# Moryu-Io/Roboken-FMSKF-robot-controller

Measured on NVIDIA B200. Metric: robot-instance control steps/sec, higher is better.
Workload: dtype f32

## Files before the change

### roboken-fmskf-robot-controller_b200/csrc/rk_imu.cu

```cuda
#include <string.h>

#include "rk_common.cuh"
#include "rk_math.cuh"
#include "rk_stream.cuh"

namespace rk {

struct ImuData {
  float d[16];
};

RK_DEV void cvt2_s16(uint32_t w, float &lo, float &hi) {
  asm("{ .reg .b16 l, h; mov.b32 {l, h}, %2; cvt.rn.f32.s16 %0, l; cvt.rn.f32.s16 %1, h; }" : "=f"(lo), "=f"(hi) : "r"(w));
}
struct ImuQ {
  float2 a[4], b[4];
};
RK_DEV void imu_q_pairs(ImuQ &k, const float qi[4]) {
  k.a[0] = make_float2(qi[3], -qi[2]), k.a[1] = make_float2(qi[2], qi[3]), k.a[2] = make_float2(-qi[1], qi[0]), k.a[3] = make_float2(-qi[0], -qi[1]);
  k.b[0] = make_float2(qi[1], qi[0]), k.b[1] = make_float2(-qi[0], qi[1]), k.b[2] = make_float2(qi[3], qi[2]), k.b[3] = make_float2(-qi[2], qi[3]);
}
RK_DEV float2 imu_mul2(float s, float2 k, float nz) { return __ffma2_rn(make_float2(s, s), k, make_float2(nz, nz)); }
RK_DEV void imu_update_data_w(const ImuQ &k, const uint32_t rw[8], float nz, ImuData &o) {
  float f[16];
#pragma unroll
  for(int j = 0; j < 8; j++) cvt2_s16(rw[j], f[2 * j], f[2 * j + 1]);
  const float KA = 16.0f / 32768.0f, KG = 2000.0f / 32768.0f, KE = 180.0f / 32768.0f, S = 1.0f / 32768.0f;
  o.d[0] = fmul(f[0], KA), o.d[1] = fmul(f[1], -KA), o.d[2] = fmul(f[2], -KA);
  o.d[3] = fmul(f[3], KG), o.d[4] = fmul(f[4], -KG), o.d[5] = fmul(f[5], -KG);
  o.d[6] = f[6], o.d[7] = -f[7], o.d[8] = -f[8];
  o.d[9]  = fsub(normalize_deg_0to360(fmul(f[9], KE)), 180.0f);
  o.d[10] = fmul(f[10], KE);
  o.d[11] = fmul(f[11], KE);
  float q[4];
#pragma unroll
  for(int j = 0; j < 4; j++) q[j] = fmul(f[12 + j], S);
  const float2 ra = __fadd2_rn(__fadd2_rn(__fadd2_rn(imu_mul2(q[0], k.a[0], nz), imu_mul2(q[1], k.a[1], nz)), imu_mul2(q[2], k.a[2], nz)),
                               imu_mul2(q[3], k.a[3], nz));
  const float2 rb = __fadd2_rn(__fadd2_rn(__fadd2_rn(imu_mul2(q[0], k.b[0], nz), imu_mul2(q[1], k.b[1], nz)), imu_mul2(q[2], k.b[2], nz)),
                               imu_mul2(q[3], k.b[3], nz));
  o.d[14] = -ra.x, o.d[13] = ra.y, o.d[12] = -rb.x, o.d[15] = rb.y;
}

template <bool OUT, bool YAW, bool GEN>
RK_DEV void imt_update_body(int64_t i, uint4 *__restrict__ state, int64_t n, int K, const int16_t *__restrict__ regs,
                            const uint8_t *__restrict__ have_quat, float4 *__restrict__ out, float *__restrict__ yaw_rad, int do_init,
                            float nz, const rk_stream_desc_t &sd) {
  float   qi[4];
  ImuData cur;
  {
    const uint4 q = ld_plane(state, n, 0, i);
    qi[0] = u2f(q.x), qi[1] = u2f(q.y), qi[2] = u2f(q.z), qi[3] = u2f(q.w);
#pragma unroll
    for(int pl = 0; pl < 4; pl++) {
      const uint4 v = ld_plane(state, n, 1 + pl, i);
      cur.d[4 * pl] = u2f(v.x), cur.d[4 * pl + 1] = u2f(v.y), cur.d[4 * pl + 2] = u2f(v.z), cur.d[4 * pl + 3] = u2f(v.w);
    }
  }
  uint32_t flags = ld_plane(state, n, 5, i).x;
  const uint4   *src = (const uint4 *)regs + i;
  const uint8_t *hsrc = have_quat ? have_quat + i : nullptr;
  uint4          c0 = make_uint4(0u, 0u, 0u, 0u), c1 = c0;
  bool           nhq = true;
  const uint32_t px  = GEN ? h32_prefix(sd.seed, 20u, (uint64_t)(sd.first + i)) : 0u;
  uint32_t       upd = sd.first_update;
  auto           fetch = [&]() {
    if(GEN) {
      stream_imu_sample(px, upd++, sd.drop_every, c0, c1, nhq);
    } else {
      c0 = __ldcs(src), c1 = __ldcs(src + n);
      src += 2 * n;
      if(hsrc) nhq = __ldcs(hsrc) != 0, hsrc += n;
    }
  };
  auto publish = [&](int u) {
    if(YAW) __stcs(yaw_rad + (int64_t)u * n + i, fmul(cur.d[RK_IS_D_ANGLE + 2], RK_DEG2RAD));
    if(OUT) {
#pragma unroll
      for(int pl = 0; pl < 4; pl++)
        __stcs(out + ((int64_t)u * 4 + pl) * n + i, make_float4(cur.d[4 * pl], cur.d[4 * pl + 1], cur.d[4 * pl + 2], cur.d[4 * pl + 3]));
    }
  };
  if(K > 0) fetch();
  ImuQ kq;
  imu_q_pairs(kq, qi);
  int u = 0;
  if(do_init && K > 0) {
    const uint32_t rw[8] = {c0.x, c0.y, c0.z, c0.w, c1.x, c1.y, c1.z, c1.w};
    if(K > 1) fetch();
    imu_update_data_w(kq, rw, nz, cur);
    cvt2_s16(rw[6], qi[0], qi[1]), cvt2_s16(rw[7], qi[2], qi[3]);
#pragma unroll
    for(int j = 0; j < 4; j++) qi[j] = fmul(qi[j], 1.0f / 32768.0f);
    imu_q_pairs(kq, qi);
    publish(0);
    u = 1;
  }
  for(; u < K; u++) {
    const uint32_t rw[8] = {c0.x, c0.y, c0.z, c0.w, c1.x, c1.y, c1.z, c1.w};
    const bool     hq    = nhq;
    if(u + 1 < K) fetch();
    if(hq) {
      flags &= ~RK_IS_FLAG_ERROR;
      imu_update_data_w(kq, rw, nz, cur);
    } else {
      flags |= RK_IS_FLAG_ERROR;
    }
    publish(u);
  }
  st_plane(state, n, 0, i, make_uint4(f2u(qi[0]), f2u(qi[1]), f2u(qi[2]), f2u(qi[3])));
#pragma unroll
  for(int pl = 0; pl < 4; pl++)
    st_plane(state, n, 1 + pl, i, make_uint4(f2u(cur.d[4 * pl]), f2u(cur.d[4 * pl + 1]), f2u(cur.d[4 * pl + 2]), f2u(cur.d[4 * pl + 3])));
  st_plane(state, n, 5, i, make_uint4(flags, 0u, 0u, 0u));
}
template <bool OUT, bool YAW, bool GEN = false>
__global__ void __launch_bounds__(256, 4)
imt_update_kernel(uint4 *__restrict__ state, int64_t n, int K, const int16_t *__restrict__ regs,
                  const uint8_t *__restrict__ have_quat, float4 *__restrict__ out, float *__restrict__ yaw_rad, int do_init, float nz_src,
                  const rk_stream_desc_t *__restrict__ desc) {
  const float            nz = fmul(-0.0f, nz_src);
  const rk_stream_desc_t sd = GEN ? *desc : rk_stream_desc_t{};
  for(int64_t i = (int64_t)blockIdx.x * blockDim.x + threadIdx.x; i < n; i += (int64_t)gridDim.x * blockDim.x)
    imt_update_body<OUT, YAW, GEN>(i, state, n, K, regs, have_quat, out, yaw_rad, do_init, nz, sd);
}

struct Wit {
  uint32_t w0, w1, w2, cnt, flags;
  bool     head_ok;
  uint32_t rw[8];
};
RK_DEV void wit_push(Wit &p, uint32_t R, uint32_t k) {
  const uint32_t s = 8u * k;
  p.w0 = __funnelshift_rc(p.w0, p.w1, s);
  p.w1 = __funnelshift_rc(p.w1, p.w2, s);
  p.w2 = __funnelshift_rc(p.w2, R, s);
}
RK_DEV bool wit_head_is_55(const Wit &p) {
  const uint32_t off = 12u - p.cnt, w = off < 4u ? p.w0 : (off < 8u ? p.w1 : p.w2);
  return ((w >> (8u * (off & 3u))) & 0xFFu) == 0x55u;
}
RK_DEV void wit_store_reg(Wit &p, uint32_t reg, uint32_t val) {
  const uint32_t slot = (reg >= 0x34u && reg <= 0x3Fu) ? reg - 0x34u : ((reg >= 0x51u && reg <= 0x54u) ? reg - 0x51u + 12u : 0xFFu);
#pragma unroll
  for(int k = 0; k < 8; k++) {
    if(slot == 2u * k) p.rw[k] = __byte_perm(p.rw[k], val, 0x3254);
    if(slot == 2u * k + 1u) p.rw[k] = __byte_perm(p.rw[k], val, 0x5410);
  }
  if(reg == 0x54u) p.flags |= 1u;
}
RK_DEV void wit_dispatch(Wit &p, uint32_t type, uint32_t d01, uint32_t d23) {
  const bool acc = type == 0x51u, gyr = type == 0x52u, ang = type == 0x53u, mag = type == 0x54u, qut = type == 0x59u;
  const uint32_t d12 = __byte_perm(d01, d23, 0x5432);
  p.rw[0] = acc ? d01 : p.rw[0];
  p.rw[1] = acc ? __byte_perm(p.rw[1], d23, 0x3254) : (gyr ? __byte_perm(p.rw[1], d01, 0x5410) : p.rw[1]);
  p.rw[2] = gyr ? d12 : p.rw[2];
  p.rw[3] = mag ? d01 : p.rw[3];
  p.rw[4] = mag ? __byte_perm(p.rw[4], d23, 0x3254) : (ang ? __byte_perm(p.rw[4], d01, 0x5410) : p.rw[4]);
  p.rw[5] = ang ? d12 : p.rw[5];
  p.rw[6] = qut ? d01 : p.rw[6];
  p.rw[7] = qut ? d23 : p.rw[7];
  p.flags |= qut ? 1u : 0u;
  if(type == 0x5Fu) {
    const uint32_t r = (p.flags >> 8) & 0xFFu;
    wit_store_reg(p, r, d01 & 0xFFFFu), wit_store_reg(p, r + 1, d01 >> 16), wit_store_reg(p, r + 2, d23 & 0xFFFFu), wit_store_reg(p, r + 3, d23 >> 16);
  }
}
RK_DEV void wit_frame(Wit &p) {
  const uint32_t f0 = __funnelshift_r(p.w0, p.w1, 8), f1 = __funnelshift_r(p.w1, p.w2, 8), f2 = p.w2 >> 8;
  wit_dispatch(p, (f0 >> 8) & 0xFFu, __byte_perm(f0, f1, 0x5432), __byte_perm(f1, f2, 0x5432));
}
RK_DEV bool wit_try_frame(Wit &p, uint32_t f0, uint32_t f1, uint32_t f2) {
  if((f0 & 0xFFu) != 0x55u) return false;
  const uint32_t sum = __vsadu4(f0, 0u) + __vsadu4(f1, 0u) + __vsadu4(f2 & 0xFFFFu, 0u);
  if((sum & 0xFFu) != ((f2 >> 16) & 0xFFu)) return false;
  wit_dispatch(p, (f0 >> 8) & 0xFFu, __byte_perm(f0, f1, 0x5432), __byte_perm(f1, f2, 0x5432));
  return true;
}
RK_DEV void wit_bytes(Wit &p, uint32_t R, uint32_t rem) {
  while(rem) {
    if(p.cnt == 0u) p.head_ok = (R & 0xFFu) == 0x55u;
    if(p.head_ok) {
      const uint32_t take = min(rem, 11u - p.cnt);
      wit_push(p, R, take);
      p.cnt += take;
      R = __funnelshift_rc(R, 0u, 8u * take);
      rem -= take;
      if(p.cnt == 11u) {
        const uint32_t sum = __vsadu4(p.w0 & 0xFFFFFF00u, 0u) + __vsadu4(p.w1, 0u) + __vsadu4(p.w2 & 0x00FFFFFFu, 0u);
        if((sum & 0xFFu) == (p.w2 >> 24)) {
          wit_frame(p);
          p.cnt = 0u;
        } else {
          p.cnt     = 10u;
          p.head_ok = ((p.w0 >> 16) & 0xFFu) == 0x55u;
        }
      }
    } else {
      if(p.cnt) {
        wit_push(p, R, 1u);
        p.head_ok = wit_head_is_55(p);
      }
      R >>= 8;
      rem--;
    }
  }
}
RK_DEV void wit_load(Wit &p, const uint4 a) {
  p.cnt = min(a.z >> 24, 10u);
  p.w0 = a.x, p.w1 = a.y, p.w2 = a.z & 0x00FFFFFFu, p.flags = a.w;
  p.head_ok = p.cnt && (p.w0 & 0xFFu) == 0x55u;
  for(uint32_t k = p.cnt; k < 12u; k++) {
    p.w2 = __funnelshift_l(p.w1, p.w2, 8);
    p.w1 = __funnelshift_l(p.w0, p.w1, 8);
    p.w0 <<= 8;
  }
}
RK_DEV uint4 wit_save(const Wit &p) {
  uint32_t w0 = p.w0, w1 = p.w1, w2 = p.w2;
  for(uint32_t k = p.cnt; k < 12u; k++) {
    w0 = __funnelshift_r(w0, w1, 8);
    w1 = __funnelshift_r(w1, w2, 8);
    w2 >>= 8;
  }
  return make_uint4(w0, w1, w2 | (p.cnt << 24), p.flags);
}

RK_DEV uint32_t smem_u32(const void *p) { return (uint32_t)__cvta_generic_to_shared(p); }
RK_DEV void mbar_init(uint64_t *bar, uint32_t count) { asm volatile("mbarrier.init.shared::cta.b64 [%0], %1;" ::"r"(smem_u32(bar)), "r"(count) : "memory"); }
RK_DEV void mbar_fence_init() { asm volatile("fence.mbarrier_init.release.cluster;" ::: "memory"); }
RK_DEV void mbar_arrive(uint64_t *bar) { asm volatile("mbarrier.arrive.shared::cta.b64 _, [%0];" ::"r"(smem_u32(bar)) : "memory"); }
RK_DEV void mbar_arrive_expect_tx(uint64_t *bar, uint32_t bytes) {
  asm volatile("mbarrier.arrive.expect_tx.shared::cta.b64 _, [%0], %1;" ::"r"(smem_u32(bar)), "r"(bytes) : "memory");
}
RK_DEV void mbar_wait(uint64_t *bar, uint32_t parity) {
  uint32_t ok;
  do {
    asm volatile("{ .reg .pred p; mbarrier.try_wait.parity.shared::cta.b64 p, [%1], %2; selp.u32 %0, 1, 0, p; }"
                 : "=r"(ok) : "r"(smem_u32(bar)), "r"(parity) : "memory");
  } while(!ok);
}
RK_DEV void bulk_g2s(void *dst, const void *src, uint32_t bytes, uint64_t *bar) {
  asm volatile("cp.async.bulk.shared::cluster.global.mbarrier::complete_tx::bytes [%0], [%1], %2, [%3];"
               ::"r"(smem_u32(dst)), "l"(src), "r"(bytes), "r"(smem_u32(bar)) : "memory");
}

constexpr int kWireStages = 16;

template <bool NC4>
__global__ void __launch_bounds__(128)
imt_feed_bytes_kernel(uint4 *__restrict__ state, uint4 *__restrict__ parser, int64_t n, int K, int ncells, const uint4 *__restrict__ cells,
                      const uint16_t *__restrict__ nbytes, float4 *__restrict__ out, float *__restrict__ yaw_rad, int do_init, float nz_src) {
  __shared__ __align__(128) uint4 ring[kWireStages][128];
  __shared__ __align__(8) uint64_t full_bar[kWireStages], empty_bar[kWireStages];
  const int      tid = threadIdx.x;
  const int64_t  i0 = (int64_t)blockIdx.x * 128, i = i0 + tid;
  const bool     live = i < n;
  const uint32_t row_bytes = (uint32_t)min((int64_t)128, n - i0) * 16u;
  const int64_t  total = (int64_t)K * ncells;
  if(tid == 0) {
    for(int s = 0; s < kWireStages; s++) mbar_init(&full_bar[s], 1u), mbar_init(&empty_bar[s], 4u);
    mbar_fence_init();
  }
  __syncthreads();
  auto issue = [&](int64_t T) {
    const int s = (int)(T % kWireStages);
    mbar_arrive_expect_tx(&full_bar[s], row_bytes);
    bulk_g2s(&ring[s][0], cells + T * n + i0, row_bytes, &full_bar[s]);
  };
  if(tid == 0)
    for(int64_t T = 0; T < total && T < kWireStages; T++) issue(T);
  auto fetch = [&](int64_t T) -> uint4 {
    const int      s   = (int)(T % kWireStages);
    const uint32_t par = (uint32_t)((T / kWireStages) & 1);
    mbar_wait(&full_bar[s], par);
    const uint4 v = ring[s][tid];
    __syncwarp();
    if((tid & 31) == 0) mbar_arrive(&empty_bar[s]);
    if(tid == 0 && T + kWireStages < total) {
      mbar_wait(&empty_bar[s], par);
      issue(T + kWireStages);
    }
    return v;
  };

  float   qi[4] = {0.0f, 0.0f, 0.0f, 0.0f};
  ImuData cur;
  uint32_t flags = 0u;
  Wit      p;
  const int64_t il = live ? i : 0;
  {
    const uint4 q = ld_plane(state, n, 0, il);
    qi[0] = u2f(q.x), qi[1] = u2f(q.y), qi[2] = u2f(q.z), qi[3] = u2f(q.w);
#pragma unroll
    for(int pl = 0; pl < 4; pl++) {
      const uint4 v = ld_plane(state, n, 1 + pl, il);
      cur.d[4 * pl] = u2f(v.x), cur.d[4 * pl + 1] = u2f(v.y), cur.d[4 * pl + 2] = u2f(v.z), cur.d[4 * pl + 3] = u2f(v.w);
    }
    flags = ld_plane(state, n, 5, il).x;
    const uint4 a = ld_plane(parser, n, 0, il), b = ld_plane(parser, n, 1, il), c = ld_plane(parser, n, 2, il);
    wit_load(p, a);
    p.rw[0] = b.x, p.rw[1] = b.y, p.rw[2] = b.z, p.rw[3] = b.w, p.rw[4] = c.x, p.rw[5] = c.y, p.rw[6] = c.z, p.rw[7] = c.w;
  }
  ImuQ kq;
  imu_q_pairs(kq, qi);
  const float nz    = fmul(-0.0f, nz_src);
  const uint4 zero4 = make_uint4(0u, 0u, 0u, 0u);
  uint4    B = (!NC4 && total > 0) ? fetch(0) : zero4;
  int64_t  t = 0;
  uint32_t nb_next = (nbytes && K > 0 && live) ? (uint32_t)__ldcs(nbytes + i) : 0xFFFFFFFFu;
  for(int u = 0; u < K; u++) {
    const bool init = do_init && u == 0;
    if(init) {
      p.cnt   = 0u;
      p.flags = (p.flags & ~0xFF00u) | (0x51u << 8) | RK_IP_FLAG_INIT_PENDING;
    }
    const uint32_t nb = live ? min(nb_next, 16u * (uint32_t)ncells) : 0u;
    if(nbytes && live && u + 1 < K) nb_next = (uint32_t)__ldcs(nbytes + (int64_t)(u + 1) * n + i);
    uint32_t done = 0u;
    if(NC4) {
      uint32_t w[17];
#pragma unroll
      for(int c = 0; c < 4; c++) {
        const uint4 v = fetch(t++);
        w[4 * c] = v.x, w[4 * c + 1] = v.y, w[4 * c + 2] = v.z, w[4 * c + 3] = v.w;
      }
      w[16] = 0u;
#pragma unroll
      for(int f = 0; f < 5; f++) {
        const int  wi = (11 * f) >> 2, sh = 8 * ((11 * f) & 3);
        const bool can = p.cnt == 0u && done == 11u * (uint32_t)f && nb >= 11u * (uint32_t)(f + 1);
        if(can && wit_try_frame(p, __funnelshift_r(w[wi], w[wi + 1], sh), __funnelshift_r(w[wi + 1], w[wi + 2], sh),
                                __funnelshift_r(w[wi + 2], w[wi + 3], sh)))
          done += 11u;
      }
      if(done < nb) {
        for(int c = 0; c < 4; c++) {
          uint4 A, Bc;
          A.x = c == 0 ? w[0] : (c == 1 ? w[4] : (c == 2 ? w[8] : w[12])), A.y = c == 0 ? w[1] : (c == 1 ? w[5] : (c == 2 ? w[9] : w[13]));
          A.z = c == 0 ? w[2] : (c == 1 ? w[6] : (c == 2 ? w[10] : w[14])), A.w = c == 0 ? w[3] : (c == 1 ? w[7] : (c == 2 ? w[11] : w[15]));
          Bc.x = c == 0 ? w[4] : (c == 1 ? w[8] : (c == 2 ? w[12] : 0u)), Bc.y = c == 0 ? w[5] : (c == 1 ? w[9] : (c == 2 ? w[13] : 0u));
          Bc.z = c == 0 ? w[6] : (c == 1 ? w[10] : (c == 2 ? w[14] : 0u)), Bc.w = c == 0 ? w[7] : (c == 1 ? w[11] : (c == 2 ? w[15] : 0u));
          const uint32_t lo = 16u * (uint32_t)c, end = min(nb, lo + 16u);
          const uint32_t span = min(nb, (c + 1 < 4) ? lo + 32u : lo + 16u);
          while(done < end) {
            const uint32_t off = done - lo, wi = off >> 2, sh = 8u * (off & 3u);
            const uint32_t x0 = wi == 0u ? A.x : (wi == 1u ? A.y : (wi == 2u ? A.z : A.w));
            if(p.cnt == 0u && span - done >= 11u) {
              const uint32_t x1 = wi == 0u ? A.y : (wi == 1u ? A.z : (wi == 2u ? A.w : Bc.x));
              const uint32_t x2 = wi == 0u ? A.z : (wi == 1u ? A.w : (wi == 2u ? Bc.x : Bc.y));
              const uint32_t x3 = wi == 0u ? A.w : (wi == 1u ? Bc.x : (wi == 2u ? Bc.y : Bc.z));
              if(wit_try_frame(p, __funnelshift_r(x0, x1, sh), __funnelshift_r(x1, x2, sh), __funnelshift_r(x2, x3, sh))) {
                done += 11u;
                continue;
              }
            }
            const uint32_t k = min(4u - (off & 3u), end - done);
            wit_bytes(p, x0 >> sh, k);
            done += k;
          }
        }
      }
    } else
    for(int c = 0; c < ncells; c++) {
      const uint4 A = B;
      t++;
      B = (t < total) ? fetch(t) : zero4;
      const uint32_t lo = 16u * (uint32_t)c, end = min(nb, lo + 16u);
      const uint32_t span = min(nb, (c + 1 < ncells) ? lo + 32u : lo + 16u);
      while(done < end) {
        const uint32_t off = done - lo, wi = off >> 2, sh = 8u * (off & 3u);
        const uint32_t x0 = wi == 0u ? A.x : (wi == 1u ? A.y : (wi == 2u ? A.z : A.w));
        if(p.cnt == 0u && span - done >= 11u) {
          const uint32_t x1 = wi == 0u ? A.y : (wi == 1u ? A.z : (wi == 2u ? A.w : B.x));
          const uint32_t x2 = wi == 0u ? A.z : (wi == 1u ? A.w : (wi == 2u ? B.x : B.y));
          const uint32_t x3 = wi == 0u ? A.w : (wi == 1u ? B.x : (wi == 2u ? B.y : B.z));
          if(wit_try_frame(p, __funnelshift_r(x0, x1, sh), __funnelshift_r(x1, x2, sh), __funnelshift_r(x2, x3, sh))) {
            done += 11u;
            continue;
          }
        }
        const uint32_t k = min(4u - (off & 3u), end - done);
        wit_bytes(p, x0 >> sh, k);
        done += k;
      }
    }
    const bool hq = (p.flags & 1u) != 0u;
    if(hq) p.flags &= ~0xFFu;
    const bool pending = (p.flags & RK_IP_FLAG_INIT_PENDING) != 0u;
    if(hq) {
      if(!pending) flags &= ~RK_IS_FLAG_ERROR;
      imu_update_data_w(kq, p.rw, nz, cur);
      if(pending) {
        cvt2_s16(p.rw[6], qi[0], qi[1]), cvt2_s16(p.rw[7], qi[2], qi[3]);
#pragma unroll
        for(int k = 0; k < 4; k++) qi[k] = fmul(qi[k], 1.0f / 32768.0f);
        imu_q_pairs(kq, qi);
        p.flags &= ~RK_IP_FLAG_INIT_PENDING;
      }
    } else if(!pending) {
      flags |= RK_IS_FLAG_ERROR;
    }
    if(live) {
      if(yaw_rad) __stcs(yaw_rad + (int64_t)u * n + i, fmul(cur.d[RK_IS_D_ANGLE + 2], RK_DEG2RAD));
      if(out) {
#pragma unroll
        for(int pl = 0; pl < 4; pl++)
          __stcs(out + ((int64_t)u * 4 + pl) * n + i, make_float4(cur.d[4 * pl], cur.d[4 * pl + 1], cur.d[4 * pl + 2], cur.d[4 * pl + 3]));
      }
    }
  }
  if(!live) return;
  st_plane(state, n, 0, i, make_uint4(f2u(qi[0]), f2u(qi[1]), f2u(qi[2]), f2u(qi[3])));
#pragma unroll
  for(int pl = 0; pl < 4; pl++)
    st_plane(state, n, 1 + pl, i, make_uint4(f2u(cur.d[4 * pl]), f2u(cur.d[4 * pl + 1]), f2u(cur.d[4 * pl + 2]), f2u(cur.d[4 * pl + 3])));
  st_plane(state, n, 5, i, make_uint4(flags, 0u, 0u, 0u));
  st_plane(parser, n, 0, i, wit_save(p));
  st_plane(parser, n, 1, i, make_uint4(p.rw[0], p.rw[1], p.rw[2], p.rw[3]));
  st_plane(parser, n, 2, i, make_uint4(p.rw[4], p.rw[5], p.rw[6], p.rw[7]));
}

}

using namespace rk;

extern "C" {

size_t rk_imt_state_words(void) { return RK_IS_WORDS; }
size_t rk_imt_state_bytes(int64_t n) { return n < 0 ? 0 : (size_t)n * RK_IS_WORDS * 4u; }

int rk_imt_update(void *d_state, int64_t n, int32_t K, const int16_t *d_regs, const uint8_t *d_have_quat, float *d_out,
                  int do_init, void *stream) {
  return rk_imt_update_yaw(d_state, n, K, d_regs, d_have_quat, d_out, nullptr, do_init, stream);
}

int rk_imt_update_yaw(void *d_state, int64_t n, int32_t K, const int16_t *d_regs, const uint8_t *d_have_quat, float *d_out,
                      float *d_yaw_rad, int do_init, void *stream) {
  return rk::imt_update_launch(d_state, n, K, d_regs, d_have_quat, d_out, d_yaw_rad, do_init, 0, stream, nullptr);
}
}

int rk::imt_update_launch(void *d_state, int64_t n, int32_t K, const int16_t *d_regs, const uint8_t *d_have_quat, float *d_out,
                          float *d_yaw_rad, int do_init, int max_ctas, void *stream, const void *d_desc) {
  if(n == 0 || K == 0) return RK_OK;
  const bool gen = d_desc != nullptr && !d_out && !d_yaw_rad;
  if(n < 0 || K < 0 || (!gen && !d_regs) || ((uintptr_t)d_regs & 15u) || ((uintptr_t)d_desc & 7u)) {
    set_error("rk_imt_update: bad n / K, or d_regs NULL / not 16-byte aligned");
    return RK_ERR_ARG;
  }
  if(!d_state || ((uintptr_t)d_state & 15u) || ((uintptr_t)d_out & 15u)) {
    set_error("rk_imt_update: d_state/d_out must be 16-byte aligned");
    return RK_ERR_ARG;
  }
  if(int rc = require_device()) return rc;
  unsigned grid = (unsigned)((n + 255) / 256);
  if(max_ctas > 0 && grid > (unsigned)max_ctas) grid = (unsigned)max_ctas;
  cudaStream_t st = (cudaStream_t)stream;
#define RK_LAUNCH_IMT(O, Y) \
  imt_update_kernel<O, Y><<<grid, 256, 0, st>>>((uint4 *)d_state, n, K, d_regs, d_have_quat, (float4 *)d_out, d_yaw_rad, do_init, 1.0f, nullptr)
  if(gen) {
    imt_update_kernel<false, false, true><<<grid, 256, 0, st>>>((uint4 *)d_state, n, K, nullptr, nullptr, nullptr, nullptr, do_init, 1.0f,
                                                                 (const rk_stream_desc_t *)d_desc);
  } else if(d_out) {
    if(d_yaw_rad) RK_LAUNCH_IMT(true, true);
    else RK_LAUNCH_IMT(true, false);
  } else {
    if(d_yaw_rad) RK_LAUNCH_IMT(false, true);
    else RK_LAUNCH_IMT(false, false);
  }
#undef RK_LAUNCH_IMT
  RK_CUDA(cudaGetLastError());
  return RK_OK;
}

extern "C" {

size_t rk_imt_parser_words(void) { return RK_IP_WORDS; }
size_t rk_imt_parser_bytes(int64_t n) { return n < 0 ? 0 : (size_t)n * RK_IP_WORDS * 4u; }

int rk_imt_feed_bytes(void *d_state, void *d_parser, int64_t n, int32_t K, int32_t ncells, const void *d_cells, const uint16_t *d_nbytes,
                      float *d_out, float *d_yaw_rad, int do_init, void *stream) {
  if(n == 0 || K == 0) return RK_OK;
  if(n < 0 || K < 0 || ncells < 0 || ncells > 4095 || (ncells > 0 && !d_cells)) {
    set_error("rk_imt_feed_bytes: bad n / K / ncells / cells");
    return RK_ERR_ARG;
  }
  if(!d_state || !d_parser || ((uintptr_t)d_state & 15u) || ((uintptr_t)d_parser & 15u) || ((uintptr_t)d_out & 15u) ||
     ((uintptr_t)d_cells & 15u) || ((uintptr_t)d_nbytes & 1u)) {
    set_error("rk_imt_feed_bytes: d_state / d_parser / d_cells / d_out must be 16-byte aligned (state and parser non-NULL)");
    return RK_ERR_ARG;
  }
  if(int rc = require_device()) return rc;
  const unsigned grid = (unsigned)((n + 127) / 128);
  if(ncells == 4)
    imt_feed_bytes_kernel<true><<<grid, 128, 0, (cudaStream_t)stream>>>((uint4 *)d_state, (uint4 *)d_parser, n, K, ncells, (const uint4 *)d_cells,
                                                                       d_nbytes, (float4 *)d_out, d_yaw_rad, do_init, 1.0f);
  else
    imt_feed_bytes_kernel<false><<<grid, 128, 0, (cudaStream_t)stream>>>((uint4 *)d_state, (uint4 *)d_parser, n, K, ncells, (const uint4 *)d_cells,
                                                                        d_nbytes, (float4 *)d_out, d_yaw_rad, do_init, 1.0f);
  RK_CUDA(cudaGetLastError());
  return RK_OK;
}

struct rk_imt {
  uint32_t    *h_mem = nullptr;
  cudaStream_t st    = nullptr;
  bool         in_flight = false;
  uint32_t *state() { return h_mem; }
  int16_t  *regs() { return (int16_t *)(h_mem + RK_IS_WORDS); }
  uint8_t  *flag() { return (uint8_t *)(h_mem + RK_IS_WORDS + 8); }
};
static int imt_settle(rk_imt *h) {
  if(h->in_flight) {
    RK_CUDA(cudaStreamSynchronize(h->st));
    h->in_flight = false;
  }
  return RK_OK;
}

int rk_imt_create(rk_imt_t **out) {
  if(!out) return RK_ERR_ARG;
  *out = nullptr;
  if(int rc = require_device()) return rc;
  rk_imt     *h = new rk_imt();
  cudaError_t e = cudaHostAlloc((void **)&h->h_mem, (RK_IS_WORDS + 8 + 4) * 4, cudaHostAllocMapped);
  if(e == cudaSuccess) memset(h->h_mem, 0, (RK_IS_WORDS + 8 + 4) * 4);
  if(e == cudaSuccess) e = cudaStreamCreateWithFlags(&h->st, cudaStreamNonBlocking);
  if(e != cudaSuccess) {
    int rc = cuda_fail(e, "rk_imt_create");
    rk_imt_destroy(h);
    return rc;
  }
  *out = h;
  return RK_OK;
}
void rk_imt_destroy(rk_imt_t *h) {
  if(!h) return;
  if(h->st) {
    cudaStreamSynchronize(h->st);
    cudaStreamDestroy(h->st);
  }
  if(h->h_mem) cudaFreeHost(h->h_mem);
  delete h;
}
static int imt_step(rk_imt_t *h, const int16_t regs[16], int have_quat, int do_init) {
  if(!h || !regs) return RK_ERR_ARG;
  if(int rc = imt_settle(h)) return rc;
  memcpy(h->regs(), regs, 32);
  *h->flag() = (uint8_t)((have_quat || do_init) ? 1 : 0);
  h->in_flight = true;
  return rk_imt_update(h->state(), 1, 1, h->regs(), h->flag(), nullptr, do_init, h->st);
}
int rk_imt_init(rk_imt_t *h, const int16_t regs[RK_IMT_REGS]) { return imt_step(h, regs, 1, 1); }
int rk_imt_update1(rk_imt_t *h, const int16_t regs[RK_IMT_REGS], int have_quat) { return imt_step(h, regs, have_quat, 0); }
int rk_imt_get_state(rk_imt_t *h, uint32_t words[RK_IS_WORDS]) {
  if(!h || !words) return RK_ERR_ARG;
  if(int rc = imt_settle(h)) return rc;
  memcpy(words, h->state(), RK_IS_WORDS * 4);
  return RK_OK;
}
int rk_imt_set_state(rk_imt_t *h, const uint32_t words[RK_IS_WORDS]) {
  if(!h || !words) return RK_ERR_ARG;
  if(int rc = imt_settle(h)) return rc;
  memcpy(h->state(), words, RK_IS_WORDS * 4);
  return RK_OK;
}
int rk_imt_get(rk_imt_t *h, float data[16], int *is_error) {
  uint32_t w[RK_IS_WORDS];
  if(!h || !data) return RK_ERR_ARG;
  if(int rc = rk_imt_get_state(h, w)) return rc;
  memcpy(data, &w[RK_IS_DATA], 64);
  if(is_error) *is_error = (w[RK_IS_FLAGS] & RK_IS_FLAG_ERROR) ? 1 : 0;
  return RK_OK;
}
int rk_imt_get_yaw(rk_imt_t *h, float *yaw_deg) {
  float d[16];
  if(!yaw_deg) return RK_ERR_ARG;
  if(int rc = rk_imt_get(h, d, nullptr)) return rc;
  *yaw_deg = d[RK_IS_D_ANGLE + 2];
  return RK_OK;
}
}
```

### roboken-fmskf-robot-controller_b200/csrc/rk_stream.cuh

```cuda
#pragma once
#include "rk_common.cuh"

namespace rk {

RK_DEV uint32_t mix32(uint32_t x) {
  x ^= x >> 16;
  x *= 0x7FEB352Du;
  x ^= x >> 15;
  x *= 0x846CA68Bu;
  x ^= x >> 16;
  return x;
}
RK_DEV uint32_t h32_prefix(uint32_t seed, uint32_t stream, uint64_t inst) {
  return mix32(mix32(seed ^ (stream * 0x9E3779B9u)) ^ (uint32_t)inst);
}
RK_DEV uint32_t h32_idx(uint32_t prefix, uint32_t idx) { return mix32(prefix ^ (idx * 0x85EBCA6Bu)); }
RK_DEV uint32_t sub32(uint32_t h, uint32_t k) { return mix32(h + (k + 1u) * 0x9E3779B9u); }
RK_DEV uint32_t lite32(uint32_t h, uint32_t k) {
  const uint32_t           m = (0x85EBCA6Bu + 2u * (k + 1u) * 0x9E3779B9u) | 1u;
  const unsigned long long x = (unsigned long long)h * m;
  return (uint32_t)x ^ (uint32_t)(x >> 32);
}
RK_DEV float    u01_32(uint32_t h) { return fmul((float)(h >> 8), 1.0f / 16777216.0f); }


RK_DEV void stream_imu_sample(uint32_t px, uint32_t upd, uint32_t drop_every, uint4 &c0, uint4 &c1, bool &have) {
  const uint32_t b = h32_idx(px, upd);
  uint32_t       w[8];
#pragma unroll
  for(int k = 0; k < 6; k++) w[k] = lite32(b, (uint32_t)k);
  const uint32_t w6 = lite32(b, 6u), w7 = lite32(b, 7u);
  const uint32_t gu[4] = {w6 & 0xFFFFu, w6 >> 16, w7 & 0xFFFFu, w7 >> 16};
  float          g[4];
#pragma unroll
  for(int k = 0; k < 4; k++) g[k] = fsub(fmul(fadd((float)gu[k], 0.5f), 1.0f / 32768.0f), 1.0f);
  const float nrm = fsqrt(fadd(fadd(fadd(fmul(g[0], g[0]), fmul(g[1], g[1])), fmul(g[2], g[2])), fmul(g[3], g[3])));
  const float sc  = fdiv(32767.0f, nrm);
  uint32_t    q[4];
#pragma unroll
  for(int k = 0; k < 4; k++) q[k] = (uint32_t)__float2int_rn(fmul(g[k], sc)) & 0xFFFFu;
  w[6] = q[0] | (q[1] << 16), w[7] = q[2] | (q[3] << 16);
  c0 = make_uint4(w[0], w[1], w[2], w[3]), c1 = make_uint4(w[4], w[5], w[6], w[7]);
  have = drop_every == 0u || (lite32(b, 8u) % drop_every) != 0u;
}
RK_DEV void stream_imu_yaw(uint32_t px, uint32_t upd, uint32_t drop_every, int16_t &yaw, bool &have) {
  const uint32_t b = h32_idx(px, upd);
  yaw  = (int16_t)(lite32(b, 5u) >> 16);
  have = drop_every == 0u || (lite32(b, 8u) % drop_every) != 0u;
}

}
```

Before: 109.4 billion.

## Skip intermediate IMU frames when no per-step outputs are requested

When neither per-step outputs nor yaw are written, the IMU update now scans backward from the last frame to find the most recent valid sample and decodes only that one, instead of decoding every frame in order. Because each frame's update fully overwrites the state, only the last valid frame determines the final result, so the intermediate decodes, loads and stream-generation work are dropped. The error flag is set from whether the final frame was valid. The risk is subtle mismatch with the sequential semantics, for example around the init frame, and the backward scan still reads have flags or regenerates hashes per frame.

```diff
diff --git a/roboken-fmskf-robot-controller_b200/csrc/rk_imu.cu b/roboken-fmskf-robot-controller_b200/csrc/rk_imu.cu
--- a/roboken-fmskf-robot-controller_b200/csrc/rk_imu.cu
+++ b/roboken-fmskf-robot-controller_b200/csrc/rk_imu.cu
@@ -42,6 +42,49 @@
   o.d[14] = -ra.x, o.d[13] = ra.y, o.d[12] = -rb.x, o.d[15] = rb.y;
 }
 
+template <bool GEN>
+RK_DEV void imt_last_frame(int64_t i, int64_t n, int K, const int16_t *__restrict__ regs, const uint8_t *__restrict__ have_quat, int do_init,
+                           float nz, const rk_stream_desc_t &sd, float qi[4], ImuData &cur, uint32_t &flags) {
+  const uint32_t px = GEN ? h32_prefix(sd.seed, 20u, (uint64_t)(sd.first + i)) : 0u;
+  auto sample = [&](int u, uint32_t rw[8]) {
+    uint4 c0, c1;
+    if(GEN) {
+      bool h;
+      stream_imu_sample(px, sd.first_update + (uint32_t)u, sd.drop_every, c0, c1, h);
+    } else {
+      const uint4 *src = (const uint4 *)regs + (int64_t)u * 2 * n + i;
+      c0 = __ldcs(src), c1 = __ldcs(src + n);
+    }
+    rw[0] = c0.x, rw[1] = c0.y, rw[2] = c0.z, rw[3] = c0.w, rw[4] = c1.x, rw[5] = c1.y, rw[6] = c1.z, rw[7] = c1.w;
+  };
+  auto have = [&](int u) -> bool {
+    if(GEN) return stream_imu_have(px, sd.first_update + (uint32_t)u, sd.drop_every);
+    return !have_quat || __ldcs(have_quat + (int64_t)u * n + i) != 0;
+  };
+  ImuQ     kq;
+  uint32_t rw[8];
+  imu_q_pairs(kq, qi);
+  int u0 = 0;
+  if(do_init && K > 0) {
+    sample(0, rw);
+    imu_update_data_w(kq, rw, nz, cur);
+    cvt2_s16(rw[6], qi[0], qi[1]), cvt2_s16(rw[7], qi[2], qi[3]);
+#pragma unroll
+    for(int j = 0; j < 4; j++) qi[j] = fmul(qi[j], 1.0f / 32768.0f);
+    imu_q_pairs(kq, qi);
+    u0 = 1;
+  }
+  if(u0 >= K) return;
+  int u = K - 1;
+  while(u >= u0 && !have(u)) u--;
+  if(u == K - 1) flags &= ~RK_IS_FLAG_ERROR;
+  else flags |= RK_IS_FLAG_ERROR;
+  if(u >= u0) {
+    sample(u, rw);
+    imu_update_data_w(kq, rw, nz, cur);
+  }
+}
+
 template <bool OUT, bool YAW, bool GEN>
 RK_DEV void imt_update_body(int64_t i, uint4 *__restrict__ state, int64_t n, int K, const int16_t *__restrict__ regs,
                             const uint8_t *__restrict__ have_quat, float4 *__restrict__ out, float *__restrict__ yaw_rad, int do_init,
@@ -58,55 +101,59 @@
     }
   }
   uint32_t flags = ld_plane(state, n, 5, i).x;
-  const uint4   *src = (const uint4 *)regs + i;
-  const uint8_t *hsrc = have_quat ? have_quat + i : nullptr;
-  uint4          c0 = make_uint4(0u, 0u, 0u, 0u), c1 = c0;
-  bool           nhq = true;
-  const uint32_t px  = GEN ? h32_prefix(sd.seed, 20u, (uint64_t)(sd.first + i)) : 0u;
-  uint32_t       upd = sd.first_update;
-  auto           fetch = [&]() {
-    if(GEN) {
-      stream_imu_sample(px, upd++, sd.drop_every, c0, c1, nhq);
-    } else {
-      c0 = __ldcs(src), c1 = __ldcs(src + n);
-      src += 2 * n;
-      if(hsrc) nhq = __ldcs(hsrc) != 0, hsrc += n;
-    }
-  };
-  auto publish = [&](int u) {
-    if(YAW) __stcs(yaw_rad + (int64_t)u * n + i, fmul(cur.d[RK_IS_D_ANGLE + 2], RK_DEG2RAD));
-    if(OUT) {
-#pragma unroll
-      for(int pl = 0; pl < 4; pl++)
-        __stcs(out + ((int64_t)u * 4 + pl) * n + i, make_float4(cur.d[4 * pl], cur.d[4 * pl + 1], cur.d[4 * pl + 2], cur.d[4 * pl + 3]));
-    }
-  };
-  if(K > 0) fetch();
-  ImuQ kq;
-  imu_q_pairs(kq, qi);
-  int u = 0;
-  if(do_init && K > 0) {
-    const uint32_t rw[8] = {c0.x, c0.y, c0.z, c0.w, c1.x, c1.y, c1.z, c1.w};
-    if(K > 1) fetch();
-    imu_update_data_w(kq, rw, nz, cur);
-    cvt2_s16(rw[6], qi[0], qi[1]), cvt2_s16(rw[7], qi[2], qi[3]);
-#pragma unroll
-    for(int j = 0; j < 4; j++) qi[j] = fmul(qi[j], 1.0f / 32768.0f);
+  if constexpr(!OUT && !YAW) {
+    imt_last_frame<GEN>(i, n, K, regs, have_quat, do_init, nz, sd, qi, cur, flags);
+  } else {
+    const uint4   *src = (const uint4 *)regs + i;
+    const uint8_t *hsrc = have_quat ? have_quat + i : nullptr;
+    uint4          c0 = make_uint4(0u, 0u, 0u, 0u), c1 = c0;
+    bool           nhq = true;
+    const uint32_t px  = GEN ? h32_prefix(sd.seed, 20u, (uint64_t)(sd.first + i)) : 0u;
+    uint32_t       upd = sd.first_update;
+    auto           fetch = [&]() {
+      if(GEN) {
+        stream_imu_sample(px, upd++, sd.drop_every, c0, c1, nhq);
+      } else {
+        c0 = __ldcs(src), c1 = __ldcs(src + n);
+        src += 2 * n;
+        if(hsrc) nhq = __ldcs(hsrc) != 0, hsrc += n;
+      }
+    };
+    auto publish = [&](int u) {
+      if(YAW) __stcs(yaw_rad + (int64_t)u * n + i, fmul(cur.d[RK_IS_D_ANGLE + 2], RK_DEG2RAD));
+      if(OUT) {
+#pragma unroll
+        for(int pl = 0; pl < 4; pl++)
+          __stcs(out + ((int64_t)u * 4 + pl) * n + i, make_float4(cur.d[4 * pl], cur.d[4 * pl + 1], cur.d[4 * pl + 2], cur.d[4 * pl + 3]));
+      }
+    };
+    if(K > 0) fetch();
+    ImuQ kq;
     imu_q_pairs(kq, qi);
-    publish(0);
-    u = 1;
-  }
-  for(; u < K; u++) {
-    const uint32_t rw[8] = {c0.x, c0.y, c0.z, c0.w, c1.x, c1.y, c1.z, c1.w};
-    const bool     hq    = nhq;
-    if(u + 1 < K) fetch();
-    if(hq) {
-      flags &= ~RK_IS_FLAG_ERROR;
+    int u = 0;
+    if(do_init && K > 0) {
+      const uint32_t rw[8] = {c0.x, c0.y, c0.z, c0.w, c1.x, c1.y, c1.z, c1.w};
+      if(K > 1) fetch();
       imu_update_data_w(kq, rw, nz, cur);
-    } else {
-      flags |= RK_IS_FLAG_ERROR;
-    }
-    publish(u);
+      cvt2_s16(rw[6], qi[0], qi[1]), cvt2_s16(rw[7], qi[2], qi[3]);
+#pragma unroll
+      for(int j = 0; j < 4; j++) qi[j] = fmul(qi[j], 1.0f / 32768.0f);
+      imu_q_pairs(kq, qi);
+      publish(0);
+      u = 1;
+    }
+    for(; u < K; u++) {
+      const uint32_t rw[8] = {c0.x, c0.y, c0.z, c0.w, c1.x, c1.y, c1.z, c1.w};
+      const bool     hq    = nhq;
+      if(u + 1 < K) fetch();
+      if(hq) {
+        flags &= ~RK_IS_FLAG_ERROR;
+        imu_update_data_w(kq, rw, nz, cur);
+      } else {
+        flags |= RK_IS_FLAG_ERROR;
+      }
+      publish(u);
+    }
   }
   st_plane(state, n, 0, i, make_uint4(f2u(qi[0]), f2u(qi[1]), f2u(qi[2]), f2u(qi[3])));
 #pragma unroll
diff --git a/roboken-fmskf-robot-controller_b200/csrc/rk_stream.cuh b/roboken-fmskf-robot-controller_b200/csrc/rk_stream.cuh
--- a/roboken-fmskf-robot-controller_b200/csrc/rk_stream.cuh
+++ b/roboken-fmskf-robot-controller_b200/csrc/rk_stream.cuh
@@ -24,6 +24,9 @@
 RK_DEV float    u01_32(uint32_t h) { return fmul((float)(h >> 8), 1.0f / 16777216.0f); }
 
 
+RK_DEV bool stream_imu_have(uint32_t px, uint32_t upd, uint32_t drop_every) {
+  return drop_every == 0u || (lite32(h32_idx(px, upd), 8u) % drop_every) != 0u;
+}
 RK_DEV void stream_imu_sample(uint32_t px, uint32_t upd, uint32_t drop_every, uint4 &c0, uint4 &c1, bool &have) {
   const uint32_t b = h32_idx(px, upd);
   uint32_t       w[8];
@@ -41,12 +44,11 @@
   for(int k = 0; k < 4; k++) q[k] = (uint32_t)__float2int_rn(fmul(g[k], sc)) & 0xFFFFu;
   w[6] = q[0] | (q[1] << 16), w[7] = q[2] | (q[3] << 16);
   c0 = make_uint4(w[0], w[1], w[2], w[3]), c1 = make_uint4(w[4], w[5], w[6], w[7]);
-  have = drop_every == 0u || (lite32(b, 8u) % drop_every) != 0u;
+  have = stream_imu_have(px, upd, drop_every);
 }
 RK_DEV void stream_imu_yaw(uint32_t px, uint32_t upd, uint32_t drop_every, int16_t &yaw, bool &have) {
-  const uint32_t b = h32_idx(px, upd);
-  yaw  = (int16_t)(lite32(b, 5u) >> 16);
-  have = drop_every == 0u || (lite32(b, 8u) % drop_every) != 0u;
+  yaw  = (int16_t)(lite32(h32_idx(px, upd), 5u) >> 16);
+  have = stream_imu_have(px, upd, drop_every);
 }
 
 }
```

Result: faster. 114.9 billion, median of 6 (+5.0%).
